# wesselb/stheno

Measured on AMD Instinct MI355X. Metric: GP logpdf+posterior evals/sec at N=16384 D=8 fp64, higher is better.
Workload: dtype f64; 1 GPU; EQ() kernel, N=16384 D=8 fp64, logpdf + condition, posterior mean/var at N*=2048; nan_scan=every step (the library's per-tensor memo is cleared at the start of each step), call_order=posterior-first, info_check=behind the call that factorised (the library's default), parallelism=replicas only (1 independent evals in flight, one process per GPU)

## Files before the change

### stheno_amd/csrc/gpk_potrf.hip

```cpp
#include "gpk_common.hpp"
#include "gpk_gemm_tile.hpp"
#include "gpk_potrf_pipe.hpp"
#include <vector>

namespace {

constexpr int LDP = 130;

template <typename T>
struct DiagArgs {
    T* A;
    int64_t ld, bstride, off;
    int n;
    T* dinv;
    int64_t dinv_bstride;
    int* info;
    int info_base;
    long long* prof;
    int zero_next;
    T* rhs = nullptr;
    int64_t rhs_stride = 0;
};

#define PROF_MARK(i)                                                            \
// ... 626 lines not shown
            if (tid == 0) s_ctl[0] = (int)__hip_atomic_fetch_add(p.ctrl + 2, 1u, __ATOMIC_RELAXED, __HIP_MEMORY_SCOPE_AGENT);
            __syncthreads();
            const int ft = s_ctl[0];
            __syncthreads();
            if (ft >= p.fill_tiles) {
                fill_left = false;
                continue;
            }
            int ti = 0, tj;
            const int ftn = p.fill.tiles_n, ftri = ftn * (ftn + 1) / 2;
            if (ft < ftri) {
                while ((ti + 1) * (ti + 2) / 2 <= ft) ++ti;
                tj = ft - ti * (ti + 1) / 2;
            } else {
                ti = ftn + (ft - ftri) / ftn;
                tj = (ft - ftri) % ftn;
            }
            gemm_tile<T, 128, true, true, EDGE, 1, D3_WAVES>(p.fill, ti, tj, 0, 0, smem);
            continue;
        }
        if (!panel_left) return;
        if (tid == 0) s_ctl[0] = (int)__hip_atomic_fetch_add(p.ctrl, 1u, __ATOMIC_RELAXED, __HIP_MEMORY_SCOPE_AGENT);
        __syncthreads();
        const int t = s_ctl[0];
        __syncthreads();
        if (t >= p.ntasks) {
            panel_left = false;
            continue;
        }
        while (t >= p.segoff[k + 1]) ++k;
        const PipeTask tk = pipe_decode(p.sh, k, t - p.segoff[k]);
        const int j = tk.j;
        const T* Pj = p.A + GPK_DB * j;
        const bool solve = tk.kind == PIPE_SOLVE || tk.kind == PIPE_XSOLVE;
        if (solve) {
            g.A = Pj; g.B = p.dinv + (int64_t)j * (GPK_DB * GPK_DB); g.C = const_cast<T*>(Pj); g.Cin = Pj;
            g.ldb = GPK_DB;
            g.N = GPK_DB;
            g.alpha = T(1); g.beta_over_alpha = T(0); g.has_beta = 0;
            g.tiles_n = 1;
        } else {
            g.A = Pj; g.B = Pj; g.C = p.A; g.Cin = p.A;
            g.ldb = p.ld;
            g.N = p.w;
            g.alpha = T(-1); g.beta_over_alpha = T(-1); g.has_beta = 1;
            g.tiles_n = npb;
        }
        const int s1 = 2 * (j + 1);
        if (tk.kind == PIPE_SOLVE) {
            unsigned* own = prog + (int64_t)tk.s * npb + j;
            if (!pipe_wait(p.ctrl + 16 + j, own, own, own, 1u, (unsigned)j, 0u, 0u, 2, abort_word, s_ctl)) return;
            gemm_tile<T, GPK_PIPE_STRIP, true, true, EDGE, 2, D3_WAVES, true>(g, tk.s, 0, 0, 0, smem);
            pipe_publish(own, (unsigned)(j + 1));
        } else if (tk.kind == PIPE_UPDATE) {
            unsigned* own = prog + (int64_t)tk.s * npb + j;
            unsigned* b0 = prog + (int64_t)(2 * tk.cb) * npb + j;
            const bool two = 2 * tk.cb + 1 < R;
            unsigned* piece = prog + (int64_t)tk.s * npb + tk.cb;
            if (!pipe_wait(own, b0, piece, two ? b0 + npb : own, (unsigned)(j + 1), (unsigned)(j + 1), (unsigned)j, (unsigned)(j + 1),
                           4, abort_word, s_ctl))
                return;
            gemm_tile<T, GPK_PIPE_STRIP, true, true, EDGE, 2, D3_WAVES, false>(g, tk.s, tk.cb, 0, 0, smem);
            pipe_publish(piece, (unsigned)(j + 1));
        } else if (tk.kind == PIPE_XSOLVE) {
            const int s = s1 + (tk.s >> 1);
            unsigned* own = prog + (int64_t)s * npb + j;
            if (!pipe_wait(p.ctrl + 16 + j, own, own, own, 1u, (unsigned)j, 0u, 0u, 2, abort_word, s_ctl)) return;
            long long* pf = (p.prof != nullptr && tid == 0 && tk.s == 0) ? p.prof + j * 32 : nullptr;
            if (pf) pf[17] = wall_clock64();
            gemm_tile<T, GPK_PIPE_FINE, true, true, EDGE, 4, D3_WAVES, true>(g, 4 * (j + 1) + tk.s, 0, 0, 0, smem);
            if (pf) pf[18] = wall_clock64();
            pipe_publish(own, (unsigned)(j + 1), cnt + (int64_t)s * npb + j,
                         (unsigned)pipe_xsolves_in_strip(pipe_fine_strips(p.sh, j), tk.s >> 1));
            if (pf) pf[19] = wall_clock64();
        } else {
            unsigned* b0 = prog + (int64_t)s1 * npb + j;
            const bool two = s1 + 1 < R;
            unsigned* piece = prog + (int64_t)(s1 + (tk.s >> 1)) * npb + j + 1;
            if (!pipe_wait(b0, two ? b0 + npb : b0, piece, piece, (unsigned)(j + 1), (unsigned)(j + 1), (unsigned)j, 0u, 3, abort_word, s_ctl)) return;
            long long* pf = (p.prof != nullptr && tid == 0 && tk.s == 3 && tk.cb == 1) ? p.prof + j * 32 : nullptr;
            if (pf) pf[20] = wall_clock64();
            gemm_tile<T, GPK_PIPE_FINE, true, true, EDGE, 2, D3_WAVES, false>(g, 4 * (j + 1) + tk.s, 2 * (j + 1) + tk.cb, 0, 0, smem);
            if (pf) pf[28] = wall_clock64();
            pipe_publish(nullptr, 0u, cnt + (int64_t)s1 * npb + j + 1, 0u);
            if (pf) pf[29] = wall_clock64();
        }
    }
}

template <typename T, bool EDGE>
__global__ __launch_bounds__(D3_THREADS, 2) void potrf_pipe_kernel(PipeArgs<T> p) {
    __shared__ __attribute__((aligned(16))) T S[D3_LDS_ELEMS];
    __shared__ int s_ctl[4];
    static_assert(sizeof(T) * D3_LDS_ELEMS >= 2 * 5 * op_bytes(GPK_PIPE_FINE) && sizeof(T) * D3_LDS_ELEMS >= 2 * 3 * op_bytes(GPK_PIPE_STRIP) &&
                      sizeof(T) * D3_LDS_ELEMS >= 2 * 2 * op_bytes(128),
                  "the worker's operand tiles live in the chain's block");
    if (threadIdx.x == 0) s_ctl[1] = (int)__hip_atomic_fetch_add(p.ctrl + 3, 1u, __ATOMIC_RELAXED, __HIP_MEMORY_SCOPE_AGENT);
    __syncthreads();
    const int role = s_ctl[1];
    __syncthreads();
    if (role == 0) pipe_chain<T>(p, S, s_ctl);
    else pipe_worker<T, EDGE>(p, reinterpret_cast<char*>(S), s_ctl, role);
    if (threadIdx.x == 0 && __hip_atomic_load(p.ctrl + 1, __ATOMIC_RELAXED, __HIP_MEMORY_SCOPE_AGENT) != 0u) atomicExch(p.info, -1);
}

template <typename T>
struct BatchStepArgs {
    T* A;
    int64_t ld, bstride;
    int n, batch;
    T* dinv;
    int64_t dstride;
// ... 187 lines not shown
    const T* P = x.A + cm * x.ld + c0;
    st = gpk_gemm_launch<T>(true, true, x.n - cm, ce - cm, h, T(-1), P, x.ld, x.bstride, P, x.ld, x.bstride,
                            T(1), x.A + cm * x.ld + cm, x.ld, x.bstride, x.batch, true, x.stream);
    if (st) return st;
    return potrf_panel<T>(x, cm, h);
}

template <typename T>
int potrf_panel_fused(const PanelCtx<T>& x, int64_t c0, int64_t w) {
    const int64_t ke = (c0 + w < x.n) ? c0 + w : x.n;
    for (int64_t c = c0; c < ke; c += GPK_DB) {
        const bool below = c + GPK_DB < x.n;
        DiagArgs<T> d;
        d.A = x.A; d.ld = x.ld; d.bstride = x.bstride; d.off = c; d.n = (int)x.n;
        d.dinv = x.dinv; d.dinv_bstride = x.dstride; d.info = x.info; d.info_base = x.info_base;
        d.prof = g_diag_prof;
        d.zero_next = below ? 1 : 0;
        launch_diag<T>(d, 1u, x.stream);
        GPK_CHECK_LAUNCH();
        if (!below) break;
        T* Wc = x.dinv + (c / GPK_DB) * (int64_t)(GPK_DB * GPK_DB);
        const int st = gpk_panel_step_launch<T>(x.A, x.n, x.ld, c, Wc, ke, reinterpret_cast<unsigned*>(Wc + (int64_t)GPK_DB * GPK_DB), x.stream);
        if (st) return st;
    }
    return GPK_OK;
}
GPK_KNOB(int, g_fused_step, 1);

GPK_KNOB(int, g_pipe, 1);
int g_pipe_cus = 0;
GPK_KNOB(int64_t, g_plain_nbo, 1024);
GPK_KNOB(int, g_pipe_fill, 1);
GPK_KNOB(int, g_pipe_panel_wgs, 0);

template <typename T>
int potrf_panel_pipe(const PanelCtx<T>& x, int64_t c0, int64_t w, bool* done, int64_t fill_k = 0) {
    *done = false;
    const int64_t ke = (c0 + w < x.n) ? c0 + w : x.n;
    const int64_t m = x.nrows() - c0;
    const bool last = (ke == x.n) && x.nrows() == x.n;
    PipeShape sh;
    sh.npb = (int)gpk_cdiv(ke - c0, GPK_DB);
    sh.nd = last ? sh.npb - 1 : sh.npb;
    sh.R = (int)gpk_cdiv(m, GPK_PIPE_STRIP);
    sh.R32 = (int)gpk_cdiv(m, GPK_PIPE_FINE);
    if (sh.nd < 1 || sh.npb > GPK_PIPE_MAX_BLOCKS) return GPK_OK;
    const int64_t words = pipe_ctrl_words(sh);
    if (words * (int64_t)sizeof(unsigned) > (int64_t)GPK_DB * GPK_DB * (int64_t)sizeof(T)) return GPK_OK;
    PipeArgs<T> pa;
    pa.A = x.A + c0 * x.ld + c0;
    pa.ld = x.ld;
    pa.m = (int)m;
    pa.w = (int)(ke - c0);
    pa.sh = sh;
    pa.dinv = x.dinv + (c0 / GPK_DB) * (int64_t)(GPK_DB * GPK_DB);
    pa.ctrl = reinterpret_cast<unsigned*>(pa.dinv + (int64_t)sh.nd * (GPK_DB * GPK_DB));
    pa.info = x.info;
    pa.info_off = (int)c0 + x.info_base;
    constexpr int VEC = Traits<T>::VEC;
    const bool aligned = ((uintptr_t)pa.A % 16 == 0) && ((uintptr_t)pa.dinv % 16 == 0) && (x.ld % VEC == 0);
    pa.vec_ok = aligned ? 1 : 0;
    pa.nseg = pipe_num_segments(sh);
    pa.segoff[0] = 0;
    for (int k = 0; k < pa.nseg; ++k) pa.segoff[k + 1] = pa.segoff[k] + pipe_segment_tasks(sh, k);
    for (int k = pa.nseg + 1; k <= GPK_PIPE_MAX_SEGS; ++k) pa.segoff[k] = pa.segoff[pa.nseg];
    pa.ntasks = pa.segoff[pa.nseg];
    pa.prof = g_diag_prof != nullptr ? g_diag_prof + (c0 / GPK_DB) * 32 : nullptr;
    int cus = x.max_wgs;
    if (cus <= 0) {
        if (g_pipe_cus == 0) {
            int dev = 0, v = 0;
            if (hipGetDevice(&dev) != hipSuccess || hipDeviceGetAttribute(&v, hipDeviceAttributeMultiprocessorCount, dev) != hipSuccess || v < 2)
                return GPK_ERR_LAUNCH;
            g_pipe_cus = v;
        }
        cus = g_pipe_cus;
    }
    int64_t workers = (int64_t)(pa.nseg > 4 ? pa.segoff[5] : pa.ntasks) + 4;
    if (workers > cus - 1) workers = cus - 1;
    if (workers < 1) workers = 1;
    if (pa.ntasks == 0) workers = 0;
    pa.wait_word = x.wait_word;
    pa.wait_value = x.wait_value;
    pa.fill_tiles = 0;
    pa.panel_wgs = (int)workers;
    bool fill_edge = false;
    if (fill_k > 0 && ke < x.n) {
        const int64_t mf = x.n - ke, mr = x.nrows() - ke;
        GemmArgs<T>& g = pa.fill;
        const T* P = x.A + ke * x.ld + (c0 - fill_k);
        g.A = P; g.B = P; g.C = x.A + ke * x.ld + ke; g.Cin = g.C;
        g.lda = x.ld; g.ldb = x.ld; g.ldc = x.ld; g.ldcin = x.ld;
        g.sA = g.sB = g.sC = g.sA2 = g.sB2 = g.sC2 = 0;
        g.M = (int)mr; g.N = (int)mf; g.K = (int)fill_k;
        g.alpha = T(-1); g.beta_over_alpha = T(-1); g.has_beta = 1;
        g.tiles_m = (int)gpk_cdiv(mr, 128); g.tiles_n = (int)gpk_cdiv(mf, 128);
        g.lower_only = 1; g.tri_k = 0; g.tri_k_lo = 0; g.tri_k_lo_b = 0; g.pair_cols = 0; g.colmask = 0; g.grp_tiles = 0;
        g.split_from = INT32_MAX;
        g.colscale = nullptr; g.colss = nullptr; g.ldss = 0; g.xcd_batch = 0; g.xcd_tiles = 0;
        g.vec_ok = aligned ? 1 : 0;
        fill_edge = !aligned || (mf % 128) || (mr % 128) || (fill_k % Traits<T>::BK) || g.lda >= GPK_PIPE_LD_MAX;
        pa.fill_tiles = g.tiles_n * (g.tiles_n + 1) / 2 + (g.tiles_m - g.tiles_n) * g.tiles_n;
        workers = cus - 1;
        pa.panel_wgs = g_pipe_panel_wgs > 0 ? g_pipe_panel_wgs : (cus - 1) / 3;
        if (pa.panel_wgs > workers) pa.panel_wgs = (int)workers;
    }
    if (hipMemsetAsync(pa.ctrl, 0, (size_t)words * sizeof(unsigned), x.stream) != hipSuccess) return GPK_ERR_LAUNCH;
    const bool edge = !aligned || (m % GPK_PIPE_STRIP) || ((ke - c0) % GPK_DB) || fill_edge;
    if (edge) hipLaunchKernelGGL((potrf_pipe_kernel<T, true>), dim3((unsigned)(1 + workers)), dim3(D3_THREADS), 0, x.stream, pa);
    else hipLaunchKernelGGL((potrf_pipe_kernel<T, false>), dim3((unsigned)(1 + workers)), dim3(D3_THREADS), 0, x.stream, pa);
    GPK_CHECK_LAUNCH();
// ... 240 lines not shown
    int cur = 0;
    (void)hipGetDevice(&cur);
    for (int dev = 0; dev < 64; ++dev) {
        LaDevice& d = g_la_dev[dev];
        if (d.aux == nullptr && d.priv == nullptr && d.events.empty()) continue;
        (void)hipSetDevice(dev);
        if (d.priv != nullptr) {
            (void)hipStreamSynchronize(d.priv);
            (void)hipStreamDestroy(d.priv);
        }
        for (hipEvent_t e : d.events) (void)hipEventDestroy(e);
        d = LaDevice();
    }
    (void)hipSetDevice(cur);
}

void gpk_tune_potrf(int key, int64_t value) {
    if (key == 6) GPK_KNOB_SET(g_la_min_rows = value;);
    if (key == 7) GPK_KNOB_SET(g_la_mode = (int)value;);
    if (key == 9) GPK_KNOB_SET(g_la_tail_rows = value;);
    if (key == 32) GPK_KNOB_SET(g_fused_step = (int)value;);
    if (key == 37) GPK_KNOB_SET(g_pipe = (int)value;);
    if (key == 40) GPK_KNOB_SET(g_la_fuse_diag_rows = value;);
    if (key == 41) GPK_KNOB_SET(g_la_fuse_diag_nb = (int)value;);
    if (key == 47) GPK_KNOB_SET(g_la_agg = (int)value;);
    if (key == 48) GPK_KNOB_SET(g_la_agg_min_rows = value;);
    if (key == 52) GPK_KNOB_SET(g_plain_nbo = value;);
    if (key == 53) GPK_KNOB_SET(g_batch_mixed = (int)value;);
    if (key == 54) GPK_KNOB_SET(g_batch_mixed_min = value;);
    if (key == 55) GPK_KNOB_SET(g_batch_lag = (int)value;);
    if (key == 57) GPK_KNOB_SET(g_diag_two_per_cu = (int)value;);
    if (key == 38) GPK_KNOB_SET(g_pipe_fill = (int)value;);
    if (key == 39) GPK_KNOB_SET(g_pipe_panel_wgs = (int)value;);
}

#define GPK_LA_PAD 16
int64_t gpk_potrf_la_ws_elems_impl(int64_t n, int nb) {
    return (n > nb ? n : nb) * (int64_t)(nb + GPK_LA_PAD) + (int64_t)nb * nb / 4 + 16 + 128 + nb;
}

template <typename T>
static int potrf_la_body(LaDevice* dev, T* A, int64_t n, int64_t ld, T* dinv128, T* dinv_big, int nb, int sb, T* ws, int* info,
                         hipStream_t stream, int64_t rows, int flags);

template <typename T>
int gpk_potrf_la_launch(T* A, int64_t n, int64_t ld, T* dinv128, T* dinv_big, int nb, T* ws, int* info,
                        hipStream_t stream, int sb, int64_t rows, int flags) {
    if (n <= 0) return GPK_OK;
    if (rows < n) rows = n;
    if ((flags & GPK_ROWS_RHS) && rows < n + GPK_ROWS_RHS_STRIP) return GPK_ERR_ARG(2);
    if (rows > INT32_MAX) return GPK_ERR_ARG(2);
    if (rows > n && n % GPK_DB != 0) return GPK_ERR_ARG(2);
    if (rows > n && gpk_cdiv(n, nb) > 64) return GPK_ERR_ARG(2);
    if (ld < n) return GPK_ERR_ARG(3);
    if (nb < 256 || nb > 4096 || (nb & (nb - 1))) return GPK_ERR_ARG(6);
    if (sb <= 0) sb = nb;
    if (sb < 256 || sb > nb || (sb & (sb - 1))) return GPK_ERR_ARG(10);
    if (dinv128 == nullptr || dinv_big == nullptr || ws == nullptr || info == nullptr) return GPK_ERR_ARG(4);

    std::lock_guard<std::mutex> lock(g_la_mutex);
    LaDevice* dev = la_device();
    if (dev == nullptr) return GPK_ERR_LAUNCH;
    if (stream != nullptr) return potrf_la_body<T>(dev, A, n, ld, dinv128, dinv_big, nb, sb, ws, info, stream, rows, flags);

    if (dev->priv == nullptr && hipStreamCreateWithFlags(&dev->priv, hipStreamNonBlocking) != hipSuccess) {
        dev->priv = nullptr;
// ... 237 lines not shown
```

### stheno_amd/csrc/gpk_potrf_pipe.hpp

```cpp
#pragma once

#if defined(__HIPCC__)
#define GPK_HD __host__ __device__ __forceinline__
#else
#define GPK_HD inline
#endif

#define GPK_PIPE_MAX_BLOCKS 64
#define GPK_PIPE_MAX_SEGS (3 * GPK_PIPE_MAX_BLOCKS + 2)
#define GPK_PIPE_CTRL_HEAD 96
#define GPK_PIPE_STRIP 64
#define GPK_PIPE_FINE 32

struct PipeShape {
    int R;
    int R32;
    int npb;
    int nd;
};

enum { PIPE_SOLVE = 0, PIPE_UPDATE = 1, PIPE_XSOLVE = 2, PIPE_XUPDATE = 3 };
struct PipeTask {
    int kind, j, s, cb;
};

GPK_HD int pipe_fine_strips(const PipeShape& sh, int j) {
    if (j + 1 >= sh.npb) return 0;
    const int left = sh.R32 - 4 * (j + 1);
    return left < 0 ? 0 : (left > 4 ? 4 : left);
}
GPK_HD int pipe_xupdates(int nq) { return nq <= 0 ? 0 : (nq == 1 ? 1 : (nq == 2 ? 2 : (nq == 3 ? 4 : 6))); }
GPK_HD int pipe_crit_tasks(const PipeShape& sh, int j) {
    const int nq = pipe_fine_strips(sh, j);
    return nq + pipe_xupdates(nq);
}
GPK_HD int pipe_xsolves_in_strip(int nq, int h) {
    const int left = nq - 2 * h;
    return left < 0 ? 0 : (left > 2 ? 2 : left);
}

GPK_HD int pipe_first_strip(const PipeShape& sh, int j) { return 2 * (j + 1) + ((j + 1 < sh.npb) ? 2 : 0); }

GPK_HD int pipe_updates_of_strip(const PipeShape& sh, int j, int s) {
    if (j + 1 >= sh.npb) return 0;
    const int top = (s >> 1) < sh.npb - 1 ? (s >> 1) : sh.npb - 1;
    return top > j ? top - j : 0;
}

GPK_HD int pipe_range_solves(const PipeShape& sh, int lo, int hi) {
    if (hi > sh.R) hi = sh.R;
    return hi > lo ? hi - lo : 0;
}
GPK_HD int pipe_range_updates(const PipeShape& sh, int j, int lo, int hi) {
    if (j + 1 >= sh.npb) return 0;
    if (hi > sh.R) hi = sh.R;
    int cnt = 0;
    const int flat = 2 * (sh.npb - 1);
    int s = lo;
    for (; s < hi && s < flat; ++s) cnt += pipe_updates_of_strip(sh, j, s);
    if (s < hi) cnt += (hi - s) * (sh.npb - 1 - j);
    return cnt;
}
GPK_HD int pipe_range_tasks(const PipeShape& sh, int j, int lo, int hi) {
    return pipe_range_solves(sh, lo, hi) + pipe_range_updates(sh, j, lo, hi);
}
GPK_HD PipeTask pipe_decode_range(const PipeShape& sh, int j, int lo, int hi, int q) {
    PipeTask t;
    t.j = j;
    if (hi > sh.R) hi = sh.R;
    const int nsolve = pipe_range_solves(sh, lo, hi);
    if (q < nsolve) {
        t.kind = PIPE_SOLVE;
        t.s = lo + q;
        t.cb = -1;
        return t;
    }
    t.kind = PIPE_UPDATE;
    int u = q - nsolve;
    const int flat = 2 * (sh.npb - 1);
    int s = lo;
    for (; s < hi && s < flat; ++s) {
        const int c = pipe_updates_of_strip(sh, j, s);
        if (u < c) {
            t.s = s;
            t.cb = j + 1 + u;
            return t;
        }
        u -= c;
    }
    const int per = sh.npb - 1 - j;
    t.s = s + u / per;
    t.cb = j + 1 + u % per;
    return t;
}

GPK_HD int pipe_num_segments(const PipeShape& sh) { return 3 * sh.nd + 2; }
GPK_HD void pipe_segment(int k, int& part, int& j) {
    if (k == 0) { part = 2; j = 0; return; }
    const int g = (k - 1) / 3, r = (k - 1) % 3;
    part = r;
    j = r == 0 ? g - 1 : (r == 1 ? g : g + 1);
}
GPK_HD int pipe_segment_tasks(const PipeShape& sh, int k) {
    int part, j;
    pipe_segment(k, part, j);
    if (j < 0 || j >= sh.nd) return 0;
    const int s0 = pipe_first_strip(sh, j);
    if (part == 2) return pipe_crit_tasks(sh, j);
    if (part == 1) return pipe_range_tasks(sh, j, s0, s0 + 2);
    return pipe_range_tasks(sh, j, s0 + 2, sh.R);
}
GPK_HD PipeTask pipe_decode(const PipeShape& sh, int k, int q) {
    int part, j;
    pipe_segment(k, part, j);
    const int s0 = pipe_first_strip(sh, j);
    if (part == 1) return pipe_decode_range(sh, j, s0, s0 + 2, q);
    if (part == 0) return pipe_decode_range(sh, j, s0 + 2, sh.R, q);
    PipeTask t;
    t.j = j;
    const int nq = pipe_fine_strips(sh, j);
    if (q < nq) {
        t.kind = PIPE_XSOLVE;
        t.s = q;
        t.cb = -1;
        return t;
    }
    const int u = q - nq;
    t.kind = PIPE_XUPDATE;
    t.s = u < 2 ? u : 2 + ((u - 2) >> 1);
    t.cb = u < 2 ? 0 : ((u - 2) & 1);
    return t;
}

GPK_HD int pipe_ctrl_words(const PipeShape& sh) { return GPK_PIPE_CTRL_HEAD + 2 * sh.R * sh.npb; }
```

### stheno_amd/csrc/pipe_check.cpp

```cpp
#include <cstdio>
#include <cstdlib>
#include <vector>
#include "gpk_potrf_pipe.hpp"

static int fail(const char* what, const PipeShape& sh, const PipeTask& t) {
    std::printf("FAIL %s: R=%d R32=%d npb=%d nd=%d  task kind=%d j=%d s=%d cb=%d\n", what, sh.R, sh.R32, sh.npb, sh.nd, t.kind, t.j, t.s, t.cb);
    return 1;
}

struct Model {
    PipeShape sh;
    std::vector<int> prog, cnt;
    std::vector<int> dflag;
    int chain_j = 0;
    int& P(int s, int cb) { return prog[(size_t)s * sh.npb + cb]; }
    int& C(int s, int cb) { return cnt[(size_t)s * sh.npb + cb]; }
    void run_chain() {
        while (chain_j < sh.nd) {
            const int j = chain_j;
            if (j > 0 && C(2 * j, j) != pipe_xupdates(pipe_fine_strips(sh, j - 1))) break;
            dflag[j] = 1;
            ++chain_j;
        }
    }
};

static int check(const PipeShape& sh) {
    Model m;
    m.sh = sh;
    m.prog.assign((size_t)sh.R * sh.npb, 0);
    m.cnt.assign((size_t)sh.R * sh.npb, 0);
    m.dflag.assign(sh.npb, 0);
    const int nseg = pipe_num_segments(sh);
    long total = 0;
    for (int k = 0; k < nseg; ++k) {
        const int nt = pipe_segment_tasks(sh, k);
        for (int q = 0; q < nt; ++q) {
            const PipeTask t = pipe_decode(sh, k, q);
            ++total;
            const int j = t.j;
            if (j < 0 || j >= sh.nd) return fail("step range", sh, t);
            m.run_chain();
            const int s1 = 2 * (j + 1);
            if (t.kind == PIPE_SOLVE) {
                if (t.s < pipe_first_strip(sh, j) || t.s >= sh.R) return fail("strip range", sh, t);
                if (!m.dflag[j]) return fail("solve before the inverse", sh, t);
                if (m.P(t.s, j) != j) return fail("solve: updates missing", sh, t);
                m.P(t.s, j) = j + 1;
            } else if (t.kind == PIPE_UPDATE) {
                if (t.s < pipe_first_strip(sh, j) || t.s >= sh.R) return fail("strip range", sh, t);
                if (t.cb <= j || t.cb >= sh.npb || t.cb > (t.s >> 1)) return fail("block range", sh, t);
                if (m.P(t.s, j) != j + 1) return fail("update: own strip not solved", sh, t);
                for (int h = 0; h < 2; ++h) {
                    const int sb = 2 * t.cb + h;
                    if (sb < sh.R && m.P(sb, j) != j + 1) return fail("update: rows of the column block not solved", sh, t);
                }
                if (m.P(t.s, t.cb) != j) return fail("update: previous update missing", sh, t);
                m.P(t.s, t.cb) = j + 1;
            } else if (t.kind == PIPE_XSOLVE) {
                const int nq = pipe_fine_strips(sh, j);
                if (t.s < 0 || t.s >= nq) return fail("fine strip range", sh, t);
                const int s = s1 + (t.s >> 1);
                if (s >= sh.R) return fail("fine strip beyond the matrix", sh, t);
                if (!m.dflag[j]) return fail("xsolve before the inverse", sh, t);
                if (m.P(s, j) != j) return fail("xsolve: updates missing", sh, t);
                if (++m.C(s, j) == pipe_xsolves_in_strip(nq, t.s >> 1)) m.P(s, j) = j + 1;
            } else {
                const int nq = pipe_fine_strips(sh, j);
                if (t.s < 0 || t.s >= nq || t.cb < 0 || t.cb > (t.s >> 1)) return fail("tile range", sh, t);
                for (int h = 0; h < 2; ++h)
                    if (s1 + h < sh.R && m.P(s1 + h, j) != j + 1) return fail("xupdate: rows of the block not solved", sh, t);
                const int s = s1 + (t.s >> 1);
                if (m.P(s, j + 1) != j) return fail("xupdate: previous update missing", sh, t);
                ++m.C(s1, j + 1);
            }
        }
    }
    m.run_chain();
    if (m.chain_j != sh.nd) {
        std::printf("FAIL chain stuck at block %d: R=%d npb=%d nd=%d\n", m.chain_j, sh.R, sh.npb, sh.nd);
        return 1;
    }
    for (int j = 0; j + 1 < sh.npb && j < sh.nd; ++j)
        if (m.C(2 * (j + 1), j + 1) != pipe_xupdates(pipe_fine_strips(sh, j))) {
            std::printf("FAIL diagonal block %d incomplete: R=%d npb=%d nd=%d\n", j + 1, sh.R, sh.npb, sh.nd);
            return 1;
        }
    for (int s = 0; s < sh.R; ++s)
        for (int cb = 0; cb < sh.npb && cb <= (s >> 1); ++cb) {
            const bool diag = (s >> 1) == cb;
            int want;
            if (diag) want = cb >= 1 ? (cb - 1 < sh.nd ? cb - 1 : sh.nd) : 0;
            else if (cb < sh.nd) want = cb + 1;
            else want = sh.nd;
            if (m.P(s, cb) != want) {
                std::printf("FAIL final state: R=%d npb=%d nd=%d  piece s=%d cb=%d has %d, expected %d\n", sh.R, sh.npb, sh.nd, s, cb,
                            m.P(s, cb), want);
                return 1;
            }
        }
    return 0;
}

int main() {
    int bad = 0;
    long shapes = 0;
    for (int npb = 1; npb <= 20 && !bad; ++npb)
        for (int extra = 0; extra <= 70 && !bad; ++extra)
            for (int cut = 0; cut < 4 && !bad; ++cut) {
                PipeShape sh;
                sh.npb = npb;
                sh.R32 = 4 * npb + extra - cut;
                if (extra > 0 && cut > 0 && extra < 4) continue;
                if (sh.R32 < 4 * (npb - 1) + 1) continue;
                sh.R = (sh.R32 + 1) / 2;
                for (int nd = (npb > 1 ? npb - 1 : npb); nd <= npb && !bad; ++nd) {
                    if (nd < 1) continue;
                    if (nd == npb - 1 && extra > 0) continue;
                    sh.nd = nd;
                    bad |= check(sh);
                    ++shapes;
                }
            }
    PipeShape big{256, 512, 64, 64};
    bad |= check(big);
    PipeShape tall{512, 1024, 8, 8};
    bad |= check(tall);
    if (!bad) std::printf("pipe_check: %ld shapes OK\n", shapes + 2);
    return bad;
}
```

### stheno_amd/csrc/selftest.cpp

```cpp
#include <hip/hip_runtime.h>
#include <algorithm>
#include <chrono>
#include <cmath>
#include <cstdio>
#include <cstdlib>
#include <climits>
#include <cstring>
#include <random>
#include <string>
#include <limits>
#include <vector>
#include <atomic>
#include <functional>
#include <thread>
#include "../../include/gpk.h"

#define HIPCHK(x)                                                                       \
    do {                                                                                \
        hipError_t e = (x);                                                             \
        if (e != hipSuccess) {                                                          \
            printf("HIP error %s at %s:%d\n", hipGetErrorString(e), __FILE__, __LINE__); \
            exit(3);                                                                    \
        }                                                                               \
    } while (0)
// ... 447 lines not shown
        auto got = dB.down();
        double nu = 0, de2 = 0;
        for (int b = 0; b < batch; ++b) for (int i = 0; i < n; ++i) for (int c = 0; c < nrhs; ++c) {
            const size_t o = ((size_t)b * n + i) * ldb + c;
            if (!std::isfinite((double)got[o])) nu = INFINITY;
            nu = std::max(nu, std::fabs((double)got[o] - ref[o]));
            de2 = std::max(de2, std::fabs(ref[o]));
        }
        snprintf(nm, sizeof nm, "%s_%s n%d nrhs%d sb%d batch%d st%d/%d", pass == 0 ? "trsv" : "trsm", DT<T>::name(), n, nrhs, sb, batch, s3, s4);
        report(nm, (s3 || s4) ? INFINITY : nu / de2, DT<T>::eps * 1000);
        if (pass == 1) {
            const int64_t ldx = nrhs + 1;
            Dev<T> dX((size_t)batch * n * ldx);
            dX.up(std::vector<T>((size_t)batch * n * ldx, T(7)));
            dB.up(Bm);
            const int s5 = gpk_trsm_lower_to(DT<T>::v, dA.p, n, ld, sA, dsb.p, sb, dB.p, nrhs, ldb, (int64_t)n * ldb, dX.p, ldx, (int64_t)n * ldx, batch, nullptr);
            HIPCHK(hipDeviceSynchronize());
            auto gx = dX.down();
            double nu2 = 0;
            for (int b = 0; b < batch; ++b) for (int i = 0; i < n; ++i) {
                for (int c = 0; c < nrhs; ++c) {
                    const double g = (double)gx[((size_t)b * n + i) * ldx + c];
                    if (!std::isfinite(g)) nu2 = INFINITY;
                    nu2 = std::max(nu2, std::fabs(g - ref[((size_t)b * n + i) * ldb + c]));
                }
                if ((double)gx[((size_t)b * n + i) * ldx + nrhs] != 7.0) nu2 = INFINITY;
            }
            snprintf(nm, sizeof nm, "trsm_to_%s n%d nrhs%d sb%d batch%d st%d", DT<T>::name(), n, nrhs, sb, batch, s5);
            report(nm, s5 ? INFINITY : nu2 / de2, DT<T>::eps * 1000);
        }
    }
}
template <typename T>
static void test_potrf() {
    test_potrf_case<T>(2500, 1, 0, 1, 0, 512);
    test_potrf_case<T>(4500, 1, 0, 1, 0, 1024);
    test_potrf_case<T>(2304, 1, 0, 1, 0, 256);
    test_potrf_case<T>(4096, 1, 0, 1, 0, 2048);
    test_potrf_case<T>(700, 1, 0, 1, 0, 256);
    test_potrf_case<T>(1664, 1, 256, 1, 0, 512);
    test_potrf_case<T>(10, 1, 0, 1, 3, 128);
    test_potrf_case<T>(100, 3, 0, 2, 0, 128);
    test_potrf_case<T>(128, 1, 0, 1, 130, 128);
    test_potrf_case<T>(200, 2, 0, 3, 64, 128);
    test_potrf_case<T>(256, 1, 128, 1, 0, 256);
    test_potrf_case<T>(384, 1, 256, 8, 200, 256);
    test_potrf_case<T>(500, 2, 256, 1, 129, 512);
    test_potrf_case<T>(1024, 1, 256, 1, 256, 512);
    test_potrf_case<T>(1200, 1, 512, 4, 100, 512);
    test_potrf_case<T>(1664, 1, 256, 1, 300, 256);
    test_potrf_case<T>(700, 70, 256, 1, 0, 128);
    test_potrf_case<T>(512, 64, 128, 2, 0, 128);
    test_potrf_case<T>(1024, 64, 256, 1, 0, 128);
    test_potrf_case<T>(640, 67, 256, 1, 0, 128);
    test_potrf_case<T>(1536, 65, 512, 1, 0, 128);
    test_potrf_case<T>(2048, 72, 0, 1, 0, 128);
    test_potrf_case<T>(1152, 64, 1024, 1, 0, 128);
}


template <typename T>
static void test_update2_case(int M0, int N0, int M1, int K, int reserve, int pad) {
    const int64_t lda0 = K + pad, ldb0 = K + pad, ldcin = N0 + pad, ldc0 = N0 + 2 * pad, lda1 = K + pad, ldc1 = M1 + pad;
    auto A0 = randv<T>((size_t)M0 * lda0), B0 = randv<T>((size_t)N0 * ldb0), Cin = randv<T>((size_t)M0 * ldcin);
    auto A1 = randv<T>((size_t)M1 * lda1), C1 = randv<T>((size_t)M1 * ldc1);
    std::vector<T> C0((size_t)M0 * ldc0, (T)7);
    Dev<T> dA0(A0.size()), dB0(B0.size()), dCin(Cin.size()), dC0(C0.size()), dA1(A1.size()), dC1(C1.size());
// ... 166 lines not shown
    auto G = dA.down(), R = dR.down();
    auto x = dB.down(), x2 = dB2.down();
    size_t diff = 0;
    for (int b = 0; b < batch; ++b)
        for (int i = 0; i < n; ++i)
            for (int j = 0; j <= i; ++j) diff += G[(size_t)b * bs + (size_t)i * ld + j] != R[(size_t)b * bs + (size_t)i * ld + j];
    double num = 0, den = 0;
    bool finite = true;
    for (size_t i = 0; i < x.size(); ++i) {
        if (!std::isfinite((double)x[i])) finite = false;
        num = std::max(num, std::fabs((double)x[i] - (double)x2[i])); den = std::max(den, std::fabs((double)x2[i]));
    }
    int bad = 0;
    for (int v : info.down()) bad += v != 0;
    char nm[200];
    snprintf(nm, sizeof nm, "potrf_rhs_%s n%d batch%d st%d/%d/%d bad_info%d: factors differ in %zu entries", DT<T>::name(), n, batch, st, st2, st3, bad, diff);
    report(nm, (st || st2 || st3 || bad || diff) ? INFINITY : 0.0, DT<T>::eps);
    snprintf(nm, sizeof nm, "potrf_rhs_%s n%d batch%d: L^-1 b against gpk_trsv_lower", DT<T>::name(), n, batch);
    report(nm, (st || !finite) ? INFINITY : num / den, DT<T>::eps * 200);
}

template <typename T>
static void test_potrf_rhs() {
    test_potrf_rhs_case<T>(512, 64);
    test_potrf_rhs_case<T>(1024, 70);
    test_potrf_rhs_case<T>(2048, 64);
    test_potrf_rhs_case<T>(640, 9);
    test_potrf_rhs_case<T>(300, 5);
    test_potrf_rhs_case<T>(1024, 1);
}

template <typename T>
static void test_potrf_rows() {
    test_potrf_rows_case<T>(128, 64, 0, 0, 0);
    test_potrf_rows_case<T>(640, 200, 0, 0, 0);
    test_potrf_rows_case<T>(1024, 300, 0, 0, 0);
    test_potrf_rows_case<T>(2560, 333, 0, 0, 0);
    test_potrf_rows_case<T>(5120, 260, 0, 0, 0);
    test_potrf_rows_case<T>(3072, 300, 512, 0, 1024);
    test_potrf_rows_case<T>(3072, 300, 512, 256, 1024);
    test_potrf_rows_case<T>(4096, 520, 1024, 0, 2048, 1);
    test_potrf_rows_case<T>(4096, 130, 256, 0, 512, 3);
    test_potrf_rows_case<T>(3840, 1000, 256, 0, 100, 2);
    test_potrf_rows_case<T>(2048, 77, 256, 0, 0);
    test_potrf_rows_case<T>(2176, 130, 0, 0, 0);
    test_potrf_rows_case<T>(4224, 64, 0, 0, 0);
    test_potrf_rows_case<T>(5248, 200, 0, 0, 0);
    test_potrf_rows_case<T>(4224, 96, 1024, 0, 2048);
    test_potrf_rows_case<T>(7296, 64, 1024, 512, 3072);
    test_potrf_rows_case<T>(640, 65, 0, 0, 0, 2, 1);
    test_potrf_rows_case<T>(3072, 301, 512, 0, 1024, 2, 1);
    test_potrf_rows_case<T>(3072, 65, 512, 256, 1024, 2, 3);
    test_potrf_rows_case<T>(4096, 1, 1024, 0, 2048, 1, 1);
    test_potrf_rows_case<T>(7296, 129, 1024, 512, 3072, 2, 3);
    test_potrf_rows_case<T>(2048, 78, 256, 0, 0, 2, 3);
}

template <typename T>
static void test_lookahead() {
    for (int pass = 0; pass < 2; ++pass) {
        gpk_tune(1, pass == 0 ? 0 : ((int64_t)1 << 40));
        test_update2_case<T>(300, 200, 260, 70, 0, 0);
        test_update2_case<T>(384, 128, 512, 64, 1, 0);
        test_update2_case<T>(1000, 256, 1100, 128, 1, 2);
        test_update2_case<T>(129, 1, 5, 3, 1, 1);
    }
// ... 1683 lines not shown
```

Before: 28.88 evals/s.

## Process flat panel strips left-looking as single tasks in the Cholesky pipe

Adds a PIPE_LSTRIP task kind so strips below the deep region of the panel pipeline are handled left-looking. One task applies the accumulated update from all earlier blocks (with depth K), then the newest block's update, then the triangular solve. Before, these strips got many separate per-block update and solve tasks with progress-counter handshakes. This cuts task count and cross-workgroup synchronisation, and the worker count grows with the number of flat strips. In exchange, each lstrip task now waits on more dependencies and does serial work.

```diff
diff --git a/stheno_amd/csrc/gpk_potrf.hip b/stheno_amd/csrc/gpk_potrf.hip
--- a/stheno_amd/csrc/gpk_potrf.hip
+++ b/stheno_amd/csrc/gpk_potrf.hip
@@ -682,40 +682,71 @@
         const PipeTask tk = pipe_decode(p.sh, k, t - p.segoff[k]);
         const int j = tk.j;
         const T* Pj = p.A + GPK_DB * j;
-        const bool solve = tk.kind == PIPE_SOLVE || tk.kind == PIPE_XSOLVE;
-        if (solve) {
+        auto as_solve = [&]() {
             g.A = Pj; g.B = p.dinv + (int64_t)j * (GPK_DB * GPK_DB); g.C = const_cast<T*>(Pj); g.Cin = Pj;
             g.ldb = GPK_DB;
-            g.N = GPK_DB;
+            g.N = GPK_DB; g.K = GPK_DB;
             g.alpha = T(1); g.beta_over_alpha = T(0); g.has_beta = 0;
             g.tiles_n = 1;
-        } else {
-            g.A = Pj; g.B = Pj; g.C = p.A; g.Cin = p.A;
+        };
+        auto as_update = [&](const T* first, int depth) {
+            g.A = first; g.B = first; g.C = p.A; g.Cin = p.A;
             g.ldb = p.ld;
-            g.N = p.w;
+            g.N = p.w; g.K = depth;
             g.alpha = T(-1); g.beta_over_alpha = T(-1); g.has_beta = 1;
             g.tiles_n = npb;
-        }
+        };
         const int s1 = 2 * (j + 1);
-        if (tk.kind == PIPE_SOLVE) {
+        if (tk.kind == PIPE_SOLVE || tk.kind == PIPE_UPDATE || tk.kind == PIPE_LSTRIP) {
+            const bool lstrip = tk.kind == PIPE_LSTRIP;
             unsigned* own = prog + (int64_t)tk.s * npb + j;
-            if (!pipe_wait(p.ctrl + 16 + j, own, own, own, 1u, (unsigned)j, 0u, 0u, 2, abort_word, s_ctl)) return;
-            gemm_tile<T, GPK_PIPE_STRIP, true, true, EDGE, 2, D3_WAVES, true>(g, tk.s, 0, 0, 0, smem);
-            pipe_publish(own, (unsigned)(j + 1));
-        } else if (tk.kind == PIPE_UPDATE) {
-            unsigned* own = prog + (int64_t)tk.s * npb + j;
-            unsigned* b0 = prog + (int64_t)(2 * tk.cb) * npb + j;
-            const bool two = 2 * tk.cb + 1 < R;
-            unsigned* piece = prog + (int64_t)tk.s * npb + tk.cb;
-            if (!pipe_wait(own, b0, piece, two ? b0 + npb : own, (unsigned)(j + 1), (unsigned)(j + 1), (unsigned)j, (unsigned)(j + 1),
-                           4, abort_word, s_ctl))
-                return;
-            gemm_tile<T, GPK_PIPE_STRIP, true, true, EDGE, 2, D3_WAVES, false>(g, tk.s, tk.cb, 0, 0, smem);
-            pipe_publish(piece, (unsigned)(j + 1));
+            unsigned* piece = own;
+            if (tk.kind == PIPE_SOLVE) {
+                if (!pipe_wait(p.ctrl + 16 + j, own, own, own, 1u, (unsigned)j, 0u, 0u, 2, abort_word, s_ctl)) return;
+            } else if (tk.kind == PIPE_UPDATE) {
+                unsigned* b0 = prog + (int64_t)(2 * tk.cb) * npb + j;
+                const bool two = 2 * tk.cb + 1 < R;
+                piece = prog + (int64_t)tk.s * npb + tk.cb;
+                if (!pipe_wait(own, b0, piece, two ? b0 + npb : own, (unsigned)(j + 1), (unsigned)(j + 1), (unsigned)j, (unsigned)(j + 1),
+                               4, abort_word, s_ctl))
+                    return;
+            }
+            const int nupd = lstrip ? (j >= 2 ? 2 : j) : (tk.kind == PIPE_UPDATE ? 1 : 0);
+            for (int ph = 0; ph < nupd; ++ph) {
+                if (lstrip) {
+                    if (ph + 2 == nupd) {
+                        unsigned* b0 = prog + (int64_t)(2 * j) * npb + j - 2;
+                        if (!pipe_wait(own - 2, b0, 2 * j + 1 < R ? b0 + npb : b0, own, (unsigned)(j - 1), (unsigned)(j - 1), (unsigned)(j - 1), 0u, 3,
+                                       abort_word, s_ctl))
+                            return;
+                        as_update(p.A, GPK_DB * (j - 1));
+                    } else {
+                        if (!pipe_wait(p.ctrl + 16 + j, own - 1, own, own, 1u, (unsigned)j, 0u, 0u, 2, abort_word, s_ctl)) return;
+                        as_update(Pj - GPK_DB, GPK_DB);
+                    }
+                } else {
+                    as_update(Pj, GPK_DB);
+                }
+                gemm_tile<T, GPK_PIPE_STRIP, true, true, EDGE, 2, D3_WAVES, false>(g, tk.s, lstrip ? j : tk.cb, 0, 0, smem);
+                if (lstrip) {
+                    __builtin_amdgcn_fence(__ATOMIC_RELEASE, "workgroup");
+                    gpk_barrier_stores_done();
+                    __builtin_amdgcn_fence(__ATOMIC_ACQUIRE, "workgroup");
+                } else {
+                    pipe_publish(piece, (unsigned)(j + 1));
+                }
+            }
+            if (tk.kind != PIPE_UPDATE) {
+                if (lstrip && j == 0 && !pipe_wait(p.ctrl + 16, own, own, own, 1u, 0u, 0u, 0u, 1, abort_word, s_ctl)) return;
+                as_solve();
+                gemm_tile<T, GPK_PIPE_STRIP, true, true, EDGE, 2, D3_WAVES, true>(g, tk.s, 0, 0, 0, smem);
+                pipe_publish(own, (unsigned)(j + 1));
+            }
         } else if (tk.kind == PIPE_XSOLVE) {
             const int s = s1 + (tk.s >> 1);
             unsigned* own = prog + (int64_t)s * npb + j;
             if (!pipe_wait(p.ctrl + 16 + j, own, own, own, 1u, (unsigned)j, 0u, 0u, 2, abort_word, s_ctl)) return;
+            as_solve();
             long long* pf = (p.prof != nullptr && tid == 0 && tk.s == 0) ? p.prof + j * 32 : nullptr;
             if (pf) pf[17] = wall_clock64();
             gemm_tile<T, GPK_PIPE_FINE, true, true, EDGE, 4, D3_WAVES, true>(g, 4 * (j + 1) + tk.s, 0, 0, 0, smem);
@@ -728,6 +759,7 @@
             const bool two = s1 + 1 < R;
             unsigned* piece = prog + (int64_t)(s1 + (tk.s >> 1)) * npb + j + 1;
             if (!pipe_wait(b0, two ? b0 + npb : b0, piece, piece, (unsigned)(j + 1), (unsigned)(j + 1), (unsigned)j, 0u, 3, abort_word, s_ctl)) return;
+            as_update(Pj, GPK_DB);
             long long* pf = (p.prof != nullptr && tid == 0 && tk.s == 3 && tk.cb == 1) ? p.prof + j * 32 : nullptr;
             if (pf) pf[20] = wall_clock64();
             gemm_tile<T, GPK_PIPE_FINE, true, true, EDGE, 2, D3_WAVES, false>(g, 4 * (j + 1) + tk.s, 2 * (j + 1) + tk.cb, 0, 0, smem);
@@ -981,6 +1013,7 @@
 GPK_KNOB(int64_t, g_plain_nbo, 1024);
 GPK_KNOB(int, g_pipe_fill, 1);
 GPK_KNOB(int, g_pipe_panel_wgs, 0);
+GPK_KNOB(int, g_pipe_ll, 1);
 
 template <typename T>
 int potrf_panel_pipe(const PanelCtx<T>& x, int64_t c0, int64_t w, bool* done, int64_t fill_k = 0) {
@@ -993,6 +1026,7 @@
     sh.nd = last ? sh.npb - 1 : sh.npb;
     sh.R = (int)gpk_cdiv(m, GPK_PIPE_STRIP);
     sh.R32 = (int)gpk_cdiv(m, GPK_PIPE_FINE);
+    sh.ll = g_pipe_ll ? 1 : 0;
     if (sh.nd < 1 || sh.npb > GPK_PIPE_MAX_BLOCKS) return GPK_OK;
     const int64_t words = pipe_ctrl_words(sh);
     if (words * (int64_t)sizeof(unsigned) > (int64_t)GPK_DB * GPK_DB * (int64_t)sizeof(T)) return GPK_OK;
@@ -1025,7 +1059,7 @@
         }
         cus = g_pipe_cus;
     }
-    int64_t workers = (int64_t)(pa.nseg > 4 ? pa.segoff[5] : pa.ntasks) + 4;
+    int64_t workers = (int64_t)(pa.nseg > 4 ? pa.segoff[5] : pa.ntasks) + 4 + pipe_flat_strips(sh);
     if (workers > cus - 1) workers = cus - 1;
     if (workers < 1) workers = 1;
     if (pa.ntasks == 0) workers = 0;
@@ -1332,6 +1366,7 @@
     if (key == 57) GPK_KNOB_SET(g_diag_two_per_cu = (int)value;);
     if (key == 38) GPK_KNOB_SET(g_pipe_fill = (int)value;);
     if (key == 39) GPK_KNOB_SET(g_pipe_panel_wgs = (int)value;);
+    if (key == 61) GPK_KNOB_SET(g_pipe_ll = (int)value;);
 }
 
 #define GPK_LA_PAD 16
diff --git a/stheno_amd/csrc/gpk_potrf_pipe.hpp b/stheno_amd/csrc/gpk_potrf_pipe.hpp
--- a/stheno_amd/csrc/gpk_potrf_pipe.hpp
+++ b/stheno_amd/csrc/gpk_potrf_pipe.hpp
@@ -17,12 +17,19 @@
     int R32;
     int npb;
     int nd;
+    int ll;
 };
 
-enum { PIPE_SOLVE = 0, PIPE_UPDATE = 1, PIPE_XSOLVE = 2, PIPE_XUPDATE = 3 };
+enum { PIPE_SOLVE = 0, PIPE_UPDATE = 1, PIPE_XSOLVE = 2, PIPE_XUPDATE = 3, PIPE_LSTRIP = 4 };
 struct PipeTask {
     int kind, j, s, cb;
 };
+
+GPK_HD int pipe_flat_first(const PipeShape& sh) {
+    const int f = 2 * sh.npb;
+    return (sh.ll && sh.nd == sh.npb && f < sh.R) ? f : sh.R;
+}
+GPK_HD int pipe_flat_strips(const PipeShape& sh) { return sh.R - pipe_flat_first(sh); }
 
 GPK_HD int pipe_fine_strips(const PipeShape& sh, int j) {
     if (j + 1 >= sh.npb) return 0;
@@ -48,16 +55,16 @@
 }
 
 GPK_HD int pipe_range_solves(const PipeShape& sh, int lo, int hi) {
-    if (hi > sh.R) hi = sh.R;
+    if (hi > pipe_flat_first(sh)) hi = pipe_flat_first(sh);
     return hi > lo ? hi - lo : 0;
 }
 GPK_HD int pipe_range_updates(const PipeShape& sh, int j, int lo, int hi) {
     if (j + 1 >= sh.npb) return 0;
-    if (hi > sh.R) hi = sh.R;
+    if (hi > pipe_flat_first(sh)) hi = pipe_flat_first(sh);
     int cnt = 0;
-    const int flat = 2 * (sh.npb - 1);
+    const int deep = 2 * (sh.npb - 1);
     int s = lo;
-    for (; s < hi && s < flat; ++s) cnt += pipe_updates_of_strip(sh, j, s);
+    for (; s < hi && s < deep; ++s) cnt += pipe_updates_of_strip(sh, j, s);
     if (s < hi) cnt += (hi - s) * (sh.npb - 1 - j);
     return cnt;
 }
@@ -67,7 +74,7 @@
 GPK_HD PipeTask pipe_decode_range(const PipeShape& sh, int j, int lo, int hi, int q) {
     PipeTask t;
     t.j = j;
-    if (hi > sh.R) hi = sh.R;
+    if (hi > pipe_flat_first(sh)) hi = pipe_flat_first(sh);
     const int nsolve = pipe_range_solves(sh, lo, hi);
     if (q < nsolve) {
         t.kind = PIPE_SOLVE;
@@ -77,9 +84,9 @@
     }
     t.kind = PIPE_UPDATE;
     int u = q - nsolve;
-    const int flat = 2 * (sh.npb - 1);
+    const int deep = 2 * (sh.npb - 1);
     int s = lo;
-    for (; s < hi && s < flat; ++s) {
+    for (; s < hi && s < deep; ++s) {
         const int c = pipe_updates_of_strip(sh, j, s);
         if (u < c) {
             t.s = s;
@@ -108,16 +115,23 @@
     const int s0 = pipe_first_strip(sh, j);
     if (part == 2) return pipe_crit_tasks(sh, j);
     if (part == 1) return pipe_range_tasks(sh, j, s0, s0 + 2);
-    return pipe_range_tasks(sh, j, s0 + 2, sh.R);
+    return pipe_range_tasks(sh, j, s0 + 2, sh.R) + pipe_flat_strips(sh);
 }
 GPK_HD PipeTask pipe_decode(const PipeShape& sh, int k, int q) {
     int part, j;
     pipe_segment(k, part, j);
     const int s0 = pipe_first_strip(sh, j);
     if (part == 1) return pipe_decode_range(sh, j, s0, s0 + 2, q);
-    if (part == 0) return pipe_decode_range(sh, j, s0 + 2, sh.R, q);
     PipeTask t;
     t.j = j;
+    if (part == 0) {
+        const int nsq = pipe_range_tasks(sh, j, s0 + 2, sh.R);
+        if (q < nsq) return pipe_decode_range(sh, j, s0 + 2, sh.R, q);
+        t.kind = PIPE_LSTRIP;
+        t.s = pipe_flat_first(sh) + (q - nsq);
+        t.cb = -1;
+        return t;
+    }
     const int nq = pipe_fine_strips(sh, j);
     if (q < nq) {
         t.kind = PIPE_XSOLVE;
diff --git a/stheno_amd/csrc/pipe_check.cpp b/stheno_amd/csrc/pipe_check.cpp
--- a/stheno_amd/csrc/pipe_check.cpp
+++ b/stheno_amd/csrc/pipe_check.cpp
@@ -4,17 +4,19 @@
 #include "gpk_potrf_pipe.hpp"
 
 static int fail(const char* what, const PipeShape& sh, const PipeTask& t) {
-    std::printf("FAIL %s: R=%d R32=%d npb=%d nd=%d  task kind=%d j=%d s=%d cb=%d\n", what, sh.R, sh.R32, sh.npb, sh.nd, t.kind, t.j, t.s, t.cb);
+    std::printf("FAIL %s: R=%d R32=%d npb=%d nd=%d ll=%d  task kind=%d j=%d s=%d cb=%d\n", what, sh.R, sh.R32, sh.npb, sh.nd, sh.ll, t.kind, t.j, t.s, t.cb);
     return 1;
 }
 
 struct Model {
     PipeShape sh;
     std::vector<int> prog, cnt;
+    std::vector<int> upd;
     std::vector<int> dflag;
     int chain_j = 0;
     int& P(int s, int cb) { return prog[(size_t)s * sh.npb + cb]; }
     int& C(int s, int cb) { return cnt[(size_t)s * sh.npb + cb]; }
+    int& U(int s, int cb) { return upd[(size_t)s * sh.npb + cb]; }
     void run_chain() {
         while (chain_j < sh.nd) {
             const int j = chain_j;
@@ -30,6 +32,7 @@
     m.sh = sh;
     m.prog.assign((size_t)sh.R * sh.npb, 0);
     m.cnt.assign((size_t)sh.R * sh.npb, 0);
+    m.upd.assign((size_t)sh.R * sh.npb, 0);
     m.dflag.assign(sh.npb, 0);
     const int nseg = pipe_num_segments(sh);
     long total = 0;
@@ -45,10 +48,24 @@
             if (t.kind == PIPE_SOLVE) {
                 if (t.s < pipe_first_strip(sh, j) || t.s >= sh.R) return fail("strip range", sh, t);
                 if (!m.dflag[j]) return fail("solve before the inverse", sh, t);
-                if (m.P(t.s, j) != j) return fail("solve: updates missing", sh, t);
+                if (t.s >= pipe_flat_first(sh)) return fail("solve of a flat strip", sh, t);
+                if (m.P(t.s, j) != j || m.U(t.s, j) != j) return fail("solve: updates missing", sh, t);
+                m.P(t.s, j) = j + 1;
+            } else if (t.kind == PIPE_LSTRIP) {
+                if (t.s < pipe_flat_first(sh) || t.s < 2 * sh.npb || t.s >= sh.R) return fail("lstrip: not a flat strip", sh, t);
+                if (!m.dflag[j]) return fail("lstrip before the inverse", sh, t);
+                if (j > 0 && m.P(t.s, j - 1) != j) return fail("lstrip: the strip's previous block not done", sh, t);
+                if (m.P(t.s, j) != 0 || m.U(t.s, j) != 0) return fail("lstrip: piece touched before", sh, t);
+                for (int c = 0; c < j; ++c) {
+                    if (m.P(t.s, c) != c + 1) return fail("lstrip: own column not final", sh, t);
+                    for (int h = 0; h < 2; ++h)
+                        if (2 * j + h < sh.R && m.P(2 * j + h, c) != c + 1) return fail("lstrip: rows of the block not final", sh, t);
+                }
+                m.U(t.s, j) = j;
                 m.P(t.s, j) = j + 1;
             } else if (t.kind == PIPE_UPDATE) {
                 if (t.s < pipe_first_strip(sh, j) || t.s >= sh.R) return fail("strip range", sh, t);
+                if (t.s >= pipe_flat_first(sh)) return fail("update of a flat strip", sh, t);
                 if (t.cb <= j || t.cb >= sh.npb || t.cb > (t.s >> 1)) return fail("block range", sh, t);
                 if (m.P(t.s, j) != j + 1) return fail("update: own strip not solved", sh, t);
                 for (int h = 0; h < 2; ++h) {
@@ -57,6 +74,7 @@
                 }
                 if (m.P(t.s, t.cb) != j) return fail("update: previous update missing", sh, t);
                 m.P(t.s, t.cb) = j + 1;
+                ++m.U(t.s, t.cb);
             } else if (t.kind == PIPE_XSOLVE) {
                 const int nq = pipe_fine_strips(sh, j);
                 if (t.s < 0 || t.s >= nq) return fail("fine strip range", sh, t);
@@ -65,6 +83,8 @@
                 if (!m.dflag[j]) return fail("xsolve before the inverse", sh, t);
                 if (m.P(s, j) != j) return fail("xsolve: updates missing", sh, t);
                 if (++m.C(s, j) == pipe_xsolves_in_strip(nq, t.s >> 1)) m.P(s, j) = j + 1;
+            } else if (t.kind != PIPE_XUPDATE) {
+                return fail("unknown task kind", sh, t);
             } else {
                 const int nq = pipe_fine_strips(sh, j);
                 if (t.s < 0 || t.s >= nq || t.cb < 0 || t.cb > (t.s >> 1)) return fail("tile range", sh, t);
@@ -98,13 +118,45 @@
                             m.P(s, cb), want);
                 return 1;
             }
+            const int wantu = diag ? want : (cb < sh.nd ? cb : sh.nd);
+            if (m.U(s, cb) != wantu) {
+                std::printf("FAIL final state: R=%d npb=%d nd=%d ll=%d  piece s=%d cb=%d received %d updates, expected %d\n", sh.R, sh.npb, sh.nd,
+                            sh.ll, s, cb, m.U(s, cb), wantu);
+                return 1;
+            }
         }
     return 0;
 }
 
+static int same_lists(PipeShape a) {
+    PipeShape b = a;
+    a.ll = 1; b.ll = 0;
+    const int nseg = pipe_num_segments(a);
+    for (int k = 0; k < nseg; ++k) {
+        const int nt = pipe_segment_tasks(a, k);
+        if (nt != pipe_segment_tasks(b, k)) { std::printf("FAIL lists differ without flat strips: R=%d npb=%d nd=%d segment %d\n", a.R, a.npb, a.nd, k); return 1; }
+        for (int q = 0; q < nt; ++q) {
+            const PipeTask x = pipe_decode(a, k, q), y = pipe_decode(b, k, q);
+            if (x.kind != y.kind || x.j != y.j || x.s != y.s || x.cb != y.cb) return fail("lists differ without flat strips", a, x);
+        }
+    }
+    return 0;
+}
+static int check_both(PipeShape sh, long* flat_shapes = nullptr) {
+    int bad = 0;
+    for (int ll = 1; ll >= 0 && !bad; --ll) {
+        sh.ll = ll;
+        bad |= check(sh);
+    }
+    sh.ll = 1;
+    if (pipe_flat_strips(sh) == 0) bad |= same_lists(sh);
+    else if (flat_shapes) ++*flat_shapes;
+    return bad;
+}
+
 int main() {
     int bad = 0;
-    long shapes = 0;
+    long shapes = 0, flat_shapes = 0;
     for (int npb = 1; npb <= 20 && !bad; ++npb)
         for (int extra = 0; extra <= 70 && !bad; ++extra)
             for (int cut = 0; cut < 4 && !bad; ++cut) {
@@ -118,14 +170,18 @@
                     if (nd < 1) continue;
                     if (nd == npb - 1 && extra > 0) continue;
                     sh.nd = nd;
-                    bad |= check(sh);
+                    bad |= check_both(sh, &flat_shapes);
                     ++shapes;
                 }
             }
-    PipeShape big{256, 512, 64, 64};
-    bad |= check(big);
-    PipeShape tall{512, 1024, 8, 8};
-    bad |= check(tall);
-    if (!bad) std::printf("pipe_check: %ld shapes OK\n", shapes + 2);
+    PipeShape big{256, 512, 64, 64, 1};
+    bad |= check_both(big, &flat_shapes);
+    PipeShape tall{512, 1024, 8, 8, 1};
+    bad |= check_both(tall, &flat_shapes);
+    PipeShape wide{288, 576, 32, 32, 1};
+    bad |= check_both(wide, &flat_shapes);
+    PipeShape wide_ragged{288, 575, 32, 32, 1};
+    bad |= check_both(wide_ragged, &flat_shapes);
+    if (!bad) std::printf("pipe_check: %ld shapes OK (%ld with flat strips, each as both lists)\n", shapes + 4, flat_shapes);
     return bad;
 }
diff --git a/stheno_amd/csrc/selftest.cpp b/stheno_amd/csrc/selftest.cpp
--- a/stheno_amd/csrc/selftest.cpp
+++ b/stheno_amd/csrc/selftest.cpp
@@ -503,7 +503,46 @@
     }
 }
 template <typename T>
+static void test_potrf_ll_bits_case(int n, int extra, int nbo) {
+    const int64_t ld = n, rows = (int64_t)n + extra;
+    auto A = make_spd<T>(n, 1, ld);
+    std::vector<T> full((size_t)rows * ld);
+    std::copy(A.begin(), A.end(), full.begin());
+    if (extra > 0) {
+        auto E = randv<T>((size_t)extra * ld);
+        std::copy(E.begin(), E.end(), full.begin() + (size_t)n * ld);
+    }
+    std::vector<T> got[2];
+    int st[2] = {0, 0}, inf[2] = {0, 0};
+    for (int ll = 1; ll >= 0; --ll) {
+        Dev<T> dA(full.size()), dinv((size_t)gpk_dinv_elems(n) + 128 * 128), dbig(16), ws(16);
+        Dev<int> info(1);
+        dA.up(full); info.zero();
+        gpk_tune(61, ll);
+        st[ll] = extra > 0 ? gpk_potrf_rows(DT<T>::v, dA.p, n, rows, ld, dinv.p, dbig.p, 0, 0, ws.p, info.p, nullptr)
+                           : gpk_potrf(DT<T>::v, dA.p, n, ld, 0, 1, dinv.p, info.p, nbo, nullptr);
+        HIPCHK(hipDeviceSynchronize());
+        got[ll] = dA.down();
+        inf[ll] = info.down()[0];
+    }
+    gpk_tune(61, 1);
+    size_t diff = 0;
+    bool finite = true;
+    for (int64_t i = 0; i < rows; ++i)
+        for (int64_t j = 0; j <= std::min<int64_t>(i, n - 1); ++j) {
+            const T a = got[1][(size_t)i * ld + j], b = got[0][(size_t)i * ld + j];
+            if (!std::isfinite((double)a)) finite = false;
+            diff += std::memcmp(&a, &b, sizeof(T)) != 0;
+        }
+    char nm[200];
+    snprintf(nm, sizeof nm, "potrf_ll_bits_%s n%d +%d rows nbo%d st%d/%d info%d/%d: left-looking and right-looking flat strips differ in %zu entries",
+             DT<T>::name(), n, extra, nbo, st[1], st[0], inf[1], inf[0], diff);
+    report(nm, (st[0] || st[1] || inf[0] || inf[1] || !finite || diff) ? INFINITY : 0.0, DT<T>::eps);
+}
+template <typename T>
 static void test_potrf() {
+    test_potrf_ll_bits_case<T>(640, 0, 256);
+    test_potrf_ll_bits_case<T>(600, 0, 256);
     test_potrf_case<T>(2500, 1, 0, 1, 0, 512);
     test_potrf_case<T>(4500, 1, 0, 1, 0, 1024);
     test_potrf_case<T>(2304, 1, 0, 1, 0, 256);
@@ -736,6 +775,9 @@
 
 template <typename T>
 static void test_potrf_rows() {
+    test_potrf_ll_bits_case<T>(512, 192, 0);
+    test_potrf_ll_bits_case<T>(512, 200, 0);
+    test_potrf_ll_bits_case<T>(4224, 192, 0);
     test_potrf_rows_case<T>(128, 64, 0, 0, 0);
     test_potrf_rows_case<T>(640, 200, 0, 0, 0);
     test_potrf_rows_case<T>(1024, 300, 0, 0, 0);
```

Result: no change. 28.83 evals/s (-0.2%).
